# rogeliorjr/DyCON_Paper_Replication

Hardware: AMD Instinct MI355X
Metric: train volumes/sec (96^3 patch) (higher is better)
Workload: dtype bf16

## Files before the change

### dycon_paper_replication_amd/_lib.py

```python
from __future__ import annotations

import ctypes as C
import os

_HERE = os.path.dirname(os.path.abspath(__file__))
LIB_PATH = os.environ.get("DYCON_LIB", os.path.join(_HERE, "libdycon_hip.so"))

F32, BF16 = 0, 1
CONV_1X1, CONV_K3, CONV_K2S2 = 0, 1, 2

P, I, L, F, Z, U64 = C.c_void_p, C.c_int, C.c_longlong, C.c_float, C.c_size_t, C.c_uint64

SIGNATURES = {
    "dycon_version": (I, []),
    "dycon_last_error": (C.c_char_p, []),
    "dycon_bfrag_bytes": (Z, [I, I, I, I]),
    "dycon_pack_bfrag": (I, [P, P, I, I, I, I, I, L, L, L, L, I, P]),
    "dycon_pack_batch": (I, [P, I, I, P]),
    "dycon_pack_tcn": (I, [P, P, I, I, I, I, L, L, L, L, I, P]),
    "dycon_conv_gemm_workspace": (Z, [I, I, I, I, I, I, I, I, I]),
    "dycon_conv_gemm": (I, [P, P, P, P, I, I, I, I, I, I, I, I, I, I, I, P, Z, P]),
    "dycon_conv_gemm_splits": (I, [I, I, I, I, I, I, I, I, I]),
    "dycon_conv_gemm_ex": (I, [P, P, P, P, I, I, I, I, I, I, I, I, I, I, I, P, Z, I, P]),
    "dycon_conv_direct": (I, [P, I, P, P, P, I, I, I, I, I, I, I, I, I, P]),
    "dycon_conv_wgrad_workspace": (Z, [I, I, I, I, I, I, I]),
    "dycon_conv_wgrad": (I, [P, I, P, I, P, P, I, I, I, I, I, I, I, L, L, L, P, Z, P]),
    "dycon_colsum_workspace": (Z, [L, I]),
    "dycon_colsum": (I, [P, I, P, L, I, P, Z, P]),
    "dycon_norm_workspace": (Z, [I, L, I]),
    "dycon_norm_stats": (I, [P, I, I, L, I, I, F, P, P, P, F, P, Z, P]),
    "dycon_norm_fwd": (I, [P, P, I, I, L, I, I, F, P, P, P, I, P, P, P, P, F, P, Z, P]),
    "dycon_norm_fwd_is_fused": (I, [I, L, I, I]),
    "dycon_norm_fwd_slab": (I, [P, I, P, P, P, I, I, L, I, I, F, P, P, P, I, P, P, P]),
    "dycon_norm_apply": (I, [P, P, I, I, L, I, I, P, P, P, I, P, P, P]),
    "dycon_norm_bwd": (I, [P, I, P, P, I, I, L, I, I, P, P, P, I, P, P, P, P, Z, P]),
    "dycon_norm_bwd_ex": (I, [P, I, P, P, I, I, L, I, I, P, P, P, I, P, P, P, I, P, Z, P]),
    "dycon_norm_sum_dparams": (I, [P, I, I, P, P, P]),
    "dycon_norm_head_workspace": (Z, [I, L]),
    "dycon_norm_head_fwd": (I, [P, I, I, L, I, P, P, P, I, P, P, P, P, P]),
    "dycon_norm_head_bwd": (I, [P, P, P, I, I, L, I, P, P, P, I, P, P, P, P, P, Z, P]),
    "dycon_norm_head_dparams": (I, [P, I, L, P, P, P]),
    "dycon_conv_stats_chunks": (I, [I, I, I, I, I, I, I, I]),
    "dycon_conv_gemm_stats": (I, [P, P, P, P, I, I, I, I, I, I, I, P, Z, P]),
    "dycon_norm_fwd_parts": (I, [P, P, I, I, L, I, I, F, P, P, P, I, P, P, P, P, F, P, I, P]),
    "dycon_norm_stats_parts": (I, [I, I, L, I, I, F, P, P, P, F, P, I, P]),
    "dycon_norm_bwd_ab_offset": (Z, [I, L, I]),
    "dycon_norm_bwd_stats": (I, [P, P, I, I, L, I, I, P, P, P, I, P, P, P, P, Z, P]),
    "dycon_first_block_bwd_workspace": (Z, [I, I, I, I]),
    "dycon_first_block_bwd": (I, [P, P, P, I, I, I, I, I, I, P, P, P, I, P, P, P, P, P, L, L, L, P, Z, P]),
    "dycon_conv1_wgrad_normbwd_workspace": (Z, [I, I, I, I]),
    "dycon_conv1_wgrad_normbwd": (I, [P, P, P, I, I, I, I, I, I, P, P, P, I, P, P, P, P, L, L, L, P, Z, P]),
    "dycon_norm_acc_doubles": (Z, [I, L, I]),
    "dycon_norm_fwd_acc": (I, [P, P, I, I, L, I, I, F, P, P, P, I, P, P, P, P, F, P, P]),
    "dycon_norm_bwd_acc": (I, [P, P, P, I, I, L, I, I, P, P, P, I, P, P, P, P, P, Z, P]),
    "dycon_maxpool2_fwd": (I, [P, P, P, I, I, I, I, I, I, P]),
    "dycon_maxpool2_bwd": (I, [P, P, P, I, I, I, I, I, I, P]),
    "dycon_trilinear_fwd": (I, [P, P, I, I, I, I, I, I, I, I, I, I, I, I, P]),
    "dycon_trilinear_bwd": (I, [P, P, I, I, I, I, I, I, I, I, I, I, I, I, P]),
    "dycon_copy_channels": (I, [P, I, I, P, I, I, L, I, I, P]),
    "dycon_relu_fwd": (I, [P, P, P, P, I, I, L, I, P]),
    "dycon_relu_bwd": (I, [P, P, P, P, I, I, L, I, P]),
    "dycon_scale_channels": (I, [P, P, P, I, I, L, I, P]),
    "dycon_mul_mask": (I, [P, P, F, P, I, L, P]),
    "dycon_dropout_philox": (I, [P, P, I, L, F, U64, U64, P]),
    "dycon_channel_mask_philox": (I, [P, L, F, U64, U64, P]),
    "dycon_add_noise": (I, [P, P, P, I, L, F, F, U64, U64, P]),
    "dycon_tanh": (I, [P, I, P, L, P]),
    "dycon_cast": (I, [P, I, P, I, L, P]),
    "dycon_add": (I, [P, P, P, I, L, P]),
    "dycon_seg_losses_fwd": (I, [P, P, P, I, I, I, L, F, P, I, P]),
    "dycon_seg_losses_bwd": (I, [P, P, P, I, I, I, L, F, P, P, I, P, I, P]),
    "dycon_seg_losses_finalize": (I, [P, I, I, L, F, P, P]),
    "dycon_step_loss": (I, [P, P, F, F, F, I, I, P, P, P]),
    "dycon_step_losses": (I, [P, P, I, I, L, F, C.c_double, F, I, F, F, F, I, I, P, P, P]),
    "dycon_softmax_mse_fwd": (I, [P, P, P, L, I, L, I, P]),
    "dycon_softmax_mse_bwd": (I, [P, P, P, P, L, I, L, I, P]),
    "dycon_softmax_kl_fwd": (I, [P, P, L, I, L, I, P, P, P]),
    "dycon_softmax_kl_bwd": (I, [P, P, L, I, L, I, I, P, P, P]),
    "dycon_dice_fwd": (I, [P, P, I, I, L, I, L, I, P, F, P, P, P]),
    "dycon_dice_bwd": (I, [P, P, I, I, L, I, L, I, P, F, P, P, P, P]),
    "dycon_dice1_fwd": (I, [P, P, I, L, I, L, I, P, P, P]),
    "dycon_dice1_bwd": (I, [P, P, I, L, I, L, I, P, P, P, P]),
    "dycon_entropy_fwd": (I, [P, L, I, L, F, P, P, P, P]),
    "dycon_entropy_bwd": (I, [P, L, I, L, F, P, P, P, P]),
    "dycon_sym_mse_fwd": (I, [P, P, L, P, P, P]),
    "dycon_sym_mse_bwd": (I, [P, P, L, P, P, P]),
    "dycon_kl_rows_fwd": (I, [P, L, P, L, L, L, L, I, P, P, P]),
    "dycon_kl_rows_bwd": (I, [P, L, P, L, L, L, L, I, P, P, L, P]),
    "dycon_focal_fwd": (I, [P, P, I, L, I, L, F, P, I, P, P, P]),
    "dycon_focal_bwd": (I, [P, P, I, L, I, L, F, P, I, P, P, P]),
    "dycon_l2norm_fwd": (I, [P, P, P, I, L, I, F, P]),
    "dycon_l2norm_bwd": (I, [P, P, P, P, I, L, I, F, P]),
    "dycon_mask_pool": (I, [P, I, P, I, I, I, I, I, I, I, P]),
    "dycon_fecl_workspace": (Z, [I, I, I]),
    "dycon_fecl_fwd": (I, [P, P, P, P, I, I, I, I, F, F, I, F, F, P, P, P, Z, P]),
    "dycon_fecl_finalize": (I, [P, C.c_double, F, I, P, P]),
    "dycon_set_scalars": (I, [P, I, F, F, F, F, F, F, F, F, P]),
    "dycon_fecl_bwd": (I, [P, P, P, P, I, I, I, I, F, F, I, F, F, P, P, P, P, Z, P]),
    "dycon_fecl_rows_workspace": (Z, [I, I, I]),
    "dycon_fecl_fwd_rows": (I, [P, P, P, P, I, I, I, I, F, F, P, P, Z, Z, P]),
    "dycon_fecl_gambling_finalize": (I, [P, P, I, I, I, I, P, P, P, P, Z, P, Z, P]),
    "dycon_fecl_gambling_grad": (I, [P, P, L, P, P]),
    "dycon_gambling_softmax_fwd": (I, [P, P, L, I, P]),
    "dycon_gambling_softmax_bwd": (I, [P, P, P, L, I, P]),
    "dycon_gambling_uncertainty_fwd": (I, [P, I, I, I, I, I, I, I, P, I, P]),
    "dycon_gambling_uncertainty_bwd": (I, [P, I, I, I, I, I, I, I, P, P, I, P]),
# ... 141 lines not shown
```

### dycon_paper_replication_amd/csrc/conv.hip

```cpp
#include <stdlib.h>

#include "common.h"

typedef float f32x4 __attribute__((ext_vector_type(4)));
typedef __bf16 bf16x8 __attribute__((ext_vector_type(8)));

template <typename T> struct Frag;
template <> struct Frag<float> { static constexpr int G = 4, KC = 16; };
template <> struct Frag<bf16> { static constexpr int G = 8, KC = 32; };

__device__ __forceinline__ void mma(f32x4& acc, const Vec16<float>& a, const Vec16<float>& b) {
    acc = __builtin_amdgcn_mfma_f32_16x16x4f32(a.v.x, b.v.x, acc, 0, 0, 0);
    acc = __builtin_amdgcn_mfma_f32_16x16x4f32(a.v.y, b.v.y, acc, 0, 0, 0);
    acc = __builtin_amdgcn_mfma_f32_16x16x4f32(a.v.z, b.v.z, acc, 0, 0, 0);
    acc = __builtin_amdgcn_mfma_f32_16x16x4f32(a.v.w, b.v.w, acc, 0, 0, 0);
}
__device__ __forceinline__ void mma(f32x4& acc, const Vec16<bf16>& a, const Vec16<bf16>& b) {
    acc = __builtin_amdgcn_mfma_f32_16x16x32_bf16(__builtin_bit_cast(bf16x8, a.v), __builtin_bit_cast(bf16x8, b.v),
                                                  acc, 0, 0, 0);
}

template <int MODE> __device__ __forceinline__ int n_taps() { return MODE == DYCON_CONV_K3 ? 27 : MODE == DYCON_CONV_K2S2 ? 8 : 1; }

template <int MODE>
__device__ __forceinline__ bool src_voxel(int t, int z, int y, int x, int Di, int Hi, int Wi, int& zi, int& yi, int& xi) {
    if (MODE == DYCON_CONV_K3) {
        const int dz = t / 9, dy = (t / 3) % 3, dx = t % 3;
        zi = z + dz - 1; yi = y + dy - 1; xi = x + dx - 1;
        return (unsigned)zi < (unsigned)Di && (unsigned)yi < (unsigned)Hi && (unsigned)xi < (unsigned)Wi;
    } else if (MODE == DYCON_CONV_K2S2) {
        zi = 2 * z + (t >> 2); yi = 2 * y + ((t >> 1) & 1); xi = 2 * x + (t & 1);
        return true;
    } else {
        zi = z; yi = y; xi = x;
        return true;
    }
}

template <typename T>
__global__ void pack_bfrag_kernel(const float* __restrict__ w, T* __restrict__ out, int Tn, int Cin, int N, int N0,
                                  long long s_t, long long s_c, long long s_n1, long long s_n0, int flip, int NT,
                                  long long total) {
    constexpr int G = Frag<T>::G, KC = Frag<T>::KC;
    for (long long i = (long long)blockIdx.x * blockDim.x + threadIdx.x; i < total; i += (long long)gridDim.x * blockDim.x) {
        const int e = (int)(i % G);
        long long q = i / G;
        const int lane = (int)(q % 64);
        q /= 64;
        const int nt = (int)(q % NT);
        const int kc = (int)(q / NT);
        const int k = kc * KC + G * (lane >> 4) + e;
        const int n = nt * 16 + (lane & 15);
        float v = 0.f;
        if (k < Tn * Cin && n < N) {
            int t = k / Cin;
            const int c = k - t * Cin;
            if (flip) t = Tn - 1 - t;
            v = w[t * s_t + c * s_c + (long long)(n / N0) * s_n1 + (long long)(n % N0) * s_n0];
        }
        stf(out + i, v);
    }
}

__global__ void pack_tcn_kernel(const float* __restrict__ w, float* __restrict__ out, int Tn, int Cin, int N, int N0,
                                long long s_t, long long s_c, long long s_n1, long long s_n0, int flip, long long total) {
    for (long long i = (long long)blockIdx.x * blockDim.x + threadIdx.x; i < total; i += (long long)gridDim.x * blockDim.x) {
        const int n = (int)(i % N);
        const long long q = i / N;
        const int c = (int)(q % Cin);
        int t = (int)(q / Cin);
        if (flip) t = Tn - 1 - t;
        out[i] = w[t * s_t + c * s_c + (long long)(n / N0) * s_n1 + (long long)(n % N0) * s_n0];
    }
}

__global__ __launch_bounds__(256) void pack_batch_kernel(const dycon_pack_job_t* __restrict__ jobs) {
    const dycon_pack_job_t jb = jobs[blockIdx.y];
    if (jb.kind == 2) {
        for (long long i = (long long)blockIdx.x * 256 + threadIdx.x; i < jb.total; i += (long long)gridDim.x * 256) {
            const int n = (int)(i % jb.N);
            const long long q = i / jb.N;
            const int c = (int)(q % jb.Cin);
            int t = (int)(q / jb.Cin);
            if (jb.flip) t = jb.T - 1 - t;
            ((float*)jb.out)[i] = jb.w[t * jb.s_t + c * jb.s_c + (long long)(n / jb.N0) * jb.s_n1 + (long long)(n % jb.N0) * jb.s_n0];
// ... 2440 lines not shown
    const ReduceJob j1{bias_part, bias_out, P, bias_part ? Cout : 0, 1, Cout, 0, 0, 1};
    const bool vec = L % 4 == 0 && (!bias_part || Cout % 4 == 0) && ((uintptr_t)part & 15) == 0 && (!bias_part || ((uintptr_t)bias_part & 15) == 0);
    if (vec) {
        const int nb0 = cdiv(L, 128), nb1 = bias_part ? cdiv(Cout, 128) : 0;
        reduce_partials_kernel<4><<<nb0 + nb1, 256, 0, stream>>>(j0, j1, nb0);
    } else {
        const int nb0 = cdiv(L, 32), nb1 = bias_part ? cdiv(Cout, 32) : 0;
        reduce_partials_kernel<1><<<nb0 + nb1, 256, 0, stream>>>(j0, j1, nb0);
    }
}

static void row_grid(int mode, int Di, int Hi, int Wi, int& Do, int& Ho, int& Wo) {
    if (mode == DYCON_CONV_K2S2) { Do = Di / 2; Ho = Hi / 2; Wo = Wi / 2; }
    else { Do = Di; Ho = Hi; Wo = Wi; }
}

extern "C" size_t dycon_bfrag_bytes(int dtype, int T, int Cin, int N) {
    const int KC = dtype == DYCON_BF16 ? 32 : 16, es = dtype == DYCON_BF16 ? 2 : 4;
    const long long nKC = ((long long)T * Cin + KC - 1) / KC, NT = (N + 15) / 16;
    return (size_t)(nKC * NT * 64 * (16 / es) * es);
}

extern "C" int dycon_pack_bfrag(const float* w, void* out, int dtype, int Tn, int Cin, int N, int N0, long long s_t,
                                long long s_c, long long s_n1, long long s_n0, int flip_taps, dycon_stream_t stream) {
    DYCON_REQUIRE(w && out && Tn > 0 && Cin > 0 && N > 0 && N0 > 0, "pack_bfrag: bad arguments");
    DYCON_DISPATCH(dtype, {
        constexpr int G = Frag<T>::G, KC = Frag<T>::KC;
        const int NT = (N + 15) / 16;
        const long long nKC = ((long long)Tn * Cin + KC - 1) / KC;
        const long long total = nKC * NT * 64 * G;
        const int grid = cdiv(total, 256) > 4096 ? 4096 : cdiv(total, 256);
        pack_bfrag_kernel<T><<<grid, 256, 0, stream>>>(w, (T*)out, Tn, Cin, N, N0, s_t, s_c, s_n1, s_n0, flip_taps, NT, total);
    });
    DYCON_LAUNCH_CHECK();
    return DYCON_OK;
}

extern "C" int dycon_pack_tcn(const float* w, float* out, int T, int Cin, int N, int N0, long long s_t, long long s_c,
                              long long s_n1, long long s_n0, int flip_taps, dycon_stream_t stream) {
    DYCON_REQUIRE(w && out && T > 0 && Cin > 0 && N > 0 && N0 > 0, "pack_tcn: bad arguments");
    const long long total = (long long)T * Cin * N;
    pack_tcn_kernel<<<cdiv(total, 256), 256, 0, stream>>>(w, out, T, Cin, N, N0, s_t, s_c, s_n1, s_n0, flip_taps, total);
    DYCON_LAUNCH_CHECK();
    return DYCON_OK;
}

struct SplitK { int splits, kc_per_split; };
static SplitK splitk_plan(int dtype, int mode, int scatter, long long M, int N, int Cin) {
    const int KC = dtype == DYCON_BF16 ? 32 : 16;
    const int Tn = mode == DYCON_CONV_K3 ? 27 : mode == DYCON_CONV_K2S2 ? 8 : 1;
    const int nKC = (Tn * Cin + KC - 1) / KC;
    const long long wgs = ((M + 63) / 64) * (((N + 15) / 16 + NTB - 1) / NTB);
    SplitK p{1, nKC};
    if (scatter || wgs >= 512 || nKC < 16) return p;
    long long s = (1024 + wgs - 1) / wgs;
    if (s > nKC / 6) s = nKC / 6;
    if (s < 2) return p;
    p.kc_per_split = (int)((nKC + s - 1) / s);
    p.splits = (nKC + p.kc_per_split - 1) / p.kc_per_split;
    return p;
}

static bool conv_tile_ok(int dtype, int mode, int scatter, long long DHW, int Cin, int N) {
    return dtype == DYCON_BF16 && mode == DYCON_CONV_K3 && !scatter && Cin % 32 == 0 && N % CT_BN == 0 && Cin >= 64 && DHW < 13824;
}
static SplitK conv_tile_plan(long long M, int N, int Cin) {
    constexpr long long target_wgs = 512;
    const int nKC = 27 * Cin / 32;
    const long long wgs = ((M + CT_BM - 1) / CT_BM) * (N / CT_BN);
    SplitK p{1, nKC};
    if (wgs >= 384) return p;
    long long s = target_wgs / wgs;
    if (s > nKC / 8) s = nKC / 8;
    if (s < 2) return p;
    p.kc_per_split = (int)((nKC + s - 1) / s);
    if (Cin % 64 == 0) p.kc_per_split = (p.kc_per_split + 1) & ~1;
    p.splits = (nKC + p.kc_per_split - 1) / p.kc_per_split;
    return p;
}
static bool conv_halo_ok(int dtype, int mode, int scatter, long long M, long long DHW, int Cin, int N) {
    return conv_tile_ok(dtype, mode, scatter, DHW, Cin, N) && Cin == CH_CIN && conv_tile_plan(M, N, Cin).splits <= CH_MAXS;
}

extern "C" int dycon_pack_batch(const dycon_pack_job_t* jobs_dev, int njobs, int blocks_per_job, dycon_stream_t stream) {
    DYCON_REQUIRE(jobs_dev && njobs > 0 && njobs <= 65535 && blocks_per_job > 0, "pack_batch: bad arguments");
    pack_batch_kernel<<<dim3(blocks_per_job, njobs), 256, 0, stream>>>(jobs_dev);
    DYCON_LAUNCH_CHECK();
    return DYCON_OK;
}

template <typename T, int MODE, bool SC>
static void launch_gemm(const void* x, const void* wf, const float* bias, void* y, int accumulate, int B, int Di, int Hi,
                        int Wi, int Cin, int N, int Cout, float* workspace, int defer_finish, dycon_stream_t stream) {
    int Do, Ho, Wo;
    row_grid(MODE, Di, Hi, Wi, Do, Ho, Wo);
    const long long M = (long long)B * Do * Ho * Wo;
    const int NT = (N + 15) / 16;
    const int Tn = MODE == DYCON_CONV_K3 ? 27 : MODE == DYCON_CONV_K2S2 ? 8 : 1;
    const int nKC = (Tn * Cin + Frag<T>::KC - 1) / Frag<T>::KC;
    const SplitK sk = splitk_plan(sizeof(T) == 2 ? DYCON_BF16 : DYCON_F32, MODE, SC, M, N, Cin);
    const bool split = sk.splits > 1 && workspace != nullptr;
    dim3 grid(cdiv(M, 64), cdiv(NT, NTB), split ? sk.splits : 1);
    conv_gemm_kernel<T, MODE, SC><<<grid, 256, 0, stream>>>((const T*)x, (const T*)wf, bias, (T*)y, B, Di, Hi, Wi, Cin, Do, Ho,
                                                            Wo, N, Cout, NT, nKC, accumulate, split ? workspace : nullptr,
                                                            sk.kc_per_split, split && defer_finish && N % 8 == 0);
    if (split && !defer_finish) {
        long long blocks = (M * N / 4 + 255) / 256;
        if (blocks > 2048) blocks = 2048;
        splitk_finish_kernel<T><<<(int)blocks, 256, 0, stream>>>(workspace, sk.splits, M * N, N, bias, (T*)y, accumulate);
    }
}

extern "C" size_t dycon_conv_gemm_workspace(int dtype, int mode, int scatter, int B, int Di, int Hi, int Wi, int Cin, int N) {
    int Do, Ho, Wo;
    row_grid(mode, Di, Hi, Wi, Do, Ho, Wo);
    const long long M = (long long)B * Do * Ho * Wo;
    if (conv_halo_ok(dtype, mode, scatter, M, (long long)Di * Hi * Wi, Cin, N)) return 0;
    const SplitK sk = conv_tile_ok(dtype, mode, scatter, (long long)Di * Hi * Wi, Cin, N) ? conv_tile_plan(M, N, Cin)
                                                                                       : splitk_plan(dtype, mode, scatter, M, N, Cin);
    return sk.splits > 1 ? (size_t)sk.splits * M * N * sizeof(float) : 0;
}

extern "C" int dycon_conv_gemm_splits(int dtype, int mode, int scatter, int B, int Di, int Hi, int Wi, int Cin, int N) {
    int Do, Ho, Wo;
    row_grid(mode, Di, Hi, Wi, Do, Ho, Wo);
    const long long M = (long long)B * Do * Ho * Wo;
    if (conv_halo_ok(dtype, mode, scatter, M, (long long)Di * Hi * Wi, Cin, N)) return 1;
    const SplitK sk = conv_tile_ok(dtype, mode, scatter, (long long)Di * Hi * Wi, Cin, N) ? conv_tile_plan(M, N, Cin)
                                                                                       : splitk_plan(dtype, mode, scatter, M, N, Cin);
    return sk.splits;
}

extern "C" int dycon_conv_gemm_ex(const void* x, const void* wfrag, const float* bias, void* y, int dtype, int mode,
                                  int scatter, int accumulate, int B, int Di, int Hi, int Wi, int Cin, int N, int Cout,
                                  float* workspace, size_t ws_bytes, int defer_finish, dycon_stream_t stream);

extern "C" int dycon_conv_gemm(const void* x, const void* wfrag, const float* bias, void* y, int dtype, int mode,
                               int scatter, int accumulate, int B, int Di, int Hi, int Wi, int Cin, int N, int Cout,
                               float* workspace, size_t ws_bytes, dycon_stream_t stream) {
    return dycon_conv_gemm_ex(x, wfrag, bias, y, dtype, mode, scatter, accumulate, B, Di, Hi, Wi, Cin, N, Cout, workspace, ws_bytes, 0,
                              stream);
}

static thread_local float* g_stat_part = nullptr;

static bool conv_p32_shape(int dtype, int mode, int scatter, int accumulate, int B, int Di, int Hi, int Wi, int Cin, int Cout) {
    const int nTiles = B * cdiv(Di, CL_TZ) * cdiv(Hi, CL_TY) * cdiv(Wi, CL_TX);
    return dtype == DYCON_BF16 && mode == DYCON_CONV_K3 && !scatter && !accumulate && Cin == 32 && Cout == 32 &&
           (long long)Di * Hi * Wi >= 13824 && nTiles >= 1024;
}
extern "C" int dycon_conv_stats_chunks(int dtype, int mode, int B, int Di, int Hi, int Wi, int Cin, int Cout) {
    const int nTiles = B * cdiv(Di, CL_TZ) * cdiv(Hi, CL_TY) * cdiv(Wi, CL_TX);
    if (dtype == DYCON_BF16 && mode == DYCON_CONV_K3 && Cout == 16 && (Cin == 16 || Cin == 1) && (long long)Di * Hi * Wi >= 13824)
        return 8 * min(cdiv(nTiles, 8), Cin == 16 ? 32 * P16_WGS : 128);
    if (!conv_p32_shape(dtype, mode, 0, 0, B, Di, Hi, Wi, Cin, Cout)) return 0;
    return 8 * min(cdiv(nTiles, 8), 32);
}
extern "C" int dycon_conv_gemm_ex(const void* x, const void* wfrag, const float* bias, void* y, int dtype, int mode,
                                  int scatter, int accumulate, int B, int Di, int Hi, int Wi, int Cin, int N, int Cout,
                                  float* workspace, size_t ws_bytes, int defer_finish, dycon_stream_t stream);
extern "C" int dycon_conv_gemm_stats(const void* x, const void* wfrag, const float* bias, void* y, int dtype, int B, int Di, int Hi,
                                     int Wi, int Cin, int Cout, float* stat_part, size_t stat_bytes, dycon_stream_t stream) {
    const int chunks = dycon_conv_stats_chunks(dtype, DYCON_CONV_K3, B, Di, Hi, Wi, Cin, Cout);
    DYCON_REQUIRE(chunks > 0, "conv_gemm_stats: shape not served (ask dycon_conv_stats_chunks)");
    DYCON_REQUIRE(stat_part && stat_bytes >= (size_t)B * chunks * Cout * 2 * sizeof(float), "conv_gemm_stats: statistics buffer too small");
    g_stat_part = stat_part;
    const int rc = dycon_conv_gemm_ex(x, wfrag, bias, y, dtype, DYCON_CONV_K3, 0, 0, B, Di, Hi, Wi, Cin, Cout, Cout, nullptr, 0, 0, stream);
    g_stat_part = nullptr;
    return rc;
}

extern "C" int dycon_conv_gemm_ex(const void* x, const void* wfrag, const float* bias, void* y, int dtype, int mode,
                                  int scatter, int accumulate, int B, int Di, int Hi, int Wi, int Cin, int N, int Cout,
                                  float* workspace, size_t ws_bytes, int defer_finish, dycon_stream_t stream) {
    DYCON_REQUIRE(x && wfrag && y, "conv_gemm: null pointer");
    DYCON_REQUIRE(!defer_finish || (!accumulate && workspace && dycon_conv_gemm_splits(dtype, mode, scatter, B, Di, Hi, Wi, Cin, N) > 1 &&
                                    ws_bytes >= dycon_conv_gemm_workspace(dtype, mode, scatter, B, Di, Hi, Wi, Cin, N)),
                  "conv_gemm: defer_finish needs a split-K shape, its workspace and no accumulation");
    DYCON_REQUIRE(B > 0 && Di > 0 && Hi > 0 && Wi > 0 && Cin > 0 && N > 0 && Cout > 0, "conv_gemm: bad shape");
    DYCON_REQUIRE(mode >= 0 && mode <= 2, "conv_gemm: bad mode %d", mode);
    const bool first_layer_lds = dtype == DYCON_BF16 && mode == DYCON_CONV_K3 && !scatter && Cin == 1 &&
                                 (Cout == 16 || Cout == 32 || Cout == 64) && (long long)Di * Hi * Wi >= 13824;
    DYCON_REQUIRE(first_layer_lds || Cin % (dtype == DYCON_BF16 ? 8 : 4) == 0, "conv_gemm: Cin=%d not a multiple of the fragment width", Cin);
    DYCON_REQUIRE(N % 16 == 0, "conv_gemm: N=%d not a multiple of 16 (use dycon_conv_direct)", N);
    DYCON_REQUIRE(!scatter || (mode == DYCON_CONV_1X1 && N == 8 * Cout), "conv_gemm: scatter needs mode 1x1 and N == 8*Cout");
    DYCON_REQUIRE(scatter || N == Cout, "conv_gemm: N must equal Cout without scatter");
    DYCON_REQUIRE(mode != DYCON_CONV_K2S2 || (Di % 2 == 0 && Hi % 2 == 0 && Wi % 2 == 0), "conv_gemm: k2s2 needs even dims");
    if (dtype == DYCON_BF16 && mode == DYCON_CONV_K3 && !scatter &&
        ((Cin == 1 && (Cout == 16 || Cout == 32 || Cout == 64)) ||
         ((Cin == 16 || Cin == 48 || Cin % 32 == 0) && (Cout == 16 || Cout == 32 || Cout % 64 == 0 || Cout % 48 == 0))) &&
        (long long)Di * Hi * Wi >= 13824) {
        const int tz = cdiv(Di, CL_TZ), ty = cdiv(Hi, CL_TY), tx = cdiv(Wi, CL_TX);
        const int NT = Cout / 16;
        const int ntb = Cout % 64 == 0 ? CL_NTB64 : (Cout % 48 == 0 ? 3 : NT);
        const int nTiles = B * tz * ty * tx;
        if ((Cin == 16 && Cout == 16) || (Cin == 1 && (Cout == 16 || Cout == 32 || Cout == 64))) {
            const int per_xcd = min(cdiv(nTiles, 8), Cin == 16 ? 32 * P16_WGS : 128);
            const bf16 *xp = (const bf16*)x, *wp = (const bf16*)wfrag;
            bf16* yp = (bf16*)y;
            if (Cin == 16 && accumulate) conv_k3_p16_kernel<P16_DEPTH, true><<<8 * per_xcd, 256, 0, stream>>>(xp, wp, bias, yp, B, Di, Hi, Wi, tz, ty, tx, nTiles);
            else if (Cin == 16 && g_stat_part) conv_k3_p16_kernel<P16_DEPTH, false, true><<<8 * per_xcd, 256, 0, stream>>>(xp, wp, bias, yp, B, Di, Hi, Wi, tz, ty, tx, nTiles, g_stat_part);
            else if (Cin == 16) conv_k3_p16_kernel<P16_DEPTH, false><<<8 * per_xcd, 256, 0, stream>>>(xp, wp, bias, yp, B, Di, Hi, Wi, tz, ty, tx, nTiles);
            else if (Cout == 16 && g_stat_part && !accumulate) conv_k3_c1_kernel<1, true><<<8 * per_xcd, 256, 0, stream>>>(xp, wp, bias, yp, B, Di, Hi, Wi, tz, ty, tx, nTiles, 0, g_stat_part);
            else if (Cout == 16) conv_k3_c1_kernel<1><<<8 * per_xcd, 256, 0, stream>>>(xp, wp, bias, yp, B, Di, Hi, Wi, tz, ty, tx, nTiles, accumulate);
            else if (Cout == 32) conv_k3_c1_kernel<2><<<8 * per_xcd, 256, 0, stream>>>(xp, wp, bias, yp, B, Di, Hi, Wi, tz, ty, tx, nTiles, accumulate);
            else conv_k3_c1_kernel<4><<<8 * per_xcd, 256, 0, stream>>>(xp, wp, bias, yp, B, Di, Hi, Wi, tz, ty, tx, nTiles, accumulate);
            DYCON_LAUNCH_CHECK();
            return DYCON_OK;
        }
        if (Cin == 32 && Cout == 32 && !accumulate && nTiles >= 1024) {
            const int per_xcd = min(cdiv(nTiles, 8), 32);
#define DYCON_P32(STV) conv_k3_p32_kernel<8, STV><<<8 * per_xcd, 64 * 8, 0, stream>>>((const bf16*)x, (const bf16*)wfrag, bias, (bf16*)y, B, Di, Hi, Wi, tz, ty, tx, nTiles, g_stat_part)
            if (g_stat_part) DYCON_P32(true); else DYCON_P32(false);
#undef DYCON_P32
            DYCON_LAUNCH_CHECK();
            return DYCON_OK;
        }
        dim3 grid(nTiles, NT / ntb);
#define DYCON_CL(CKV, NTBV, WMV) \
    conv_k3_lds_kernel<CKV, NTBV, WMV><<<grid, 256, 0, stream>>>((const bf16*)x, (const bf16*)wfrag, bias, (bf16*)y, B, Di, Hi, Wi, Cin, Cout, NT, tz, ty, tx, accumulate)
        if (Cin == 16 || Cin == 48) {
            if (ntb == 1) DYCON_CL(16, 1, 4); else if (ntb == 2) DYCON_CL(16, 2, 4); else if (ntb == 3) DYCON_CL(16, 3, 4); else DYCON_CL(16, 4, 2);
        } else {
            if (ntb == 1) DYCON_CL(32, 1, 4); else if (ntb == 2) DYCON_CL(32, 2, 4); else if (ntb == 3) DYCON_CL(32, 3, 4);
            else if ((long long)nTiles * (NT / ntb) <= 256)
                conv_k3_lds_kernel<32, 4, 4, 8><<<grid, 512, 0, stream>>>((const bf16*)x, (const bf16*)wfrag, bias, (bf16*)y, B, Di, Hi, Wi, Cin, Cout, NT, tz, ty, tx, accumulate);
            else DYCON_CL(32, 4, 2);
        }
#undef DYCON_CL
        DYCON_LAUNCH_CHECK();
        return DYCON_OK;
    }
    if (conv_halo_ok(dtype, mode, scatter, (long long)B * Di * Hi * Wi, (long long)Di * Hi * Wi, Cin, N)) {
        const long long M = (long long)B * Di * Hi * Wi;
        const int tz = cdiv(Di, CH_T), ty = cdiv(Hi, CH_T), tx = cdiv(Wi, CH_T);
        const SplitK sk = conv_tile_plan(M, N, Cin);
        const dim3 grid(B * tz * ty * tx, N / 64);
#define DYCON_CH(NJV) conv_k3_halo_kernel<NJV><<<grid, 64 * CH_NW, 0, stream>>>((const bf16*)x, (const bf16*)wfrag, bias, (bf16*)y, Di, Hi, Wi, N, N / 16, tz, ty, tx, sk.splits, sk.kc_per_split, accumulate)
        if (sk.splits > 2) DYCON_CH(2); else DYCON_CH(1);
#undef DYCON_CH
        DYCON_LAUNCH_CHECK();
        return DYCON_OK;
    }
    if (conv_tile_ok(dtype, mode, scatter, (long long)Di * Hi * Wi, Cin, N)) {
        const long long M = (long long)B * Di * Hi * Wi;
        const int NT = N / 16, nKC = 27 * Cin / 32;
        SplitK sk = conv_tile_plan(M, N, Cin);
        const bool split = sk.splits > 1 && workspace && ws_bytes >= (size_t)sk.splits * M * N * sizeof(float);
        dim3 grid(cdiv(M, CT_BM), N / CT_BN, split ? sk.splits : 1);
        const int layout = split && defer_finish ? 1 : 0;
        if (Cin % 64 == 0 && sk.kc_per_split % 2 == 0)
            conv_k3_tile_kernel<2><<<grid, 256, 0, stream>>>((const bf16*)x, (const bf16*)wfrag, bias, (bf16*)y, split ? workspace : nullptr, B,
                                                             Di, Hi, Wi, Cin, N, NT, nKC, sk.kc_per_split, accumulate, layout);
        else
            conv_k3_tile_kernel<1><<<grid, 256, 0, stream>>>((const bf16*)x, (const bf16*)wfrag, bias, (bf16*)y, split ? workspace : nullptr, B,
                                                             Di, Hi, Wi, Cin, N, NT, nKC, sk.kc_per_split, accumulate, layout);
        DYCON_LAUNCH_CHECK();
        if (split && !defer_finish) {
            long long blocks = (M * N / 4 + 255) / 256;
            if (blocks > 2048) blocks = 2048;
            splitk_finish_kernel<bf16><<<(int)blocks, 256, 0, stream>>>(workspace, sk.splits, M * N, N, bias, (bf16*)y, accumulate);
            DYCON_LAUNCH_CHECK();
        }
        return DYCON_OK;
    }
    float* ws = (workspace && ws_bytes >= dycon_conv_gemm_workspace(dtype, mode, scatter, B, Di, Hi, Wi, Cin, N)) ? workspace : nullptr;
    DYCON_DISPATCH(dtype, {
        if (scatter) launch_gemm<T, DYCON_CONV_1X1, true>(x, wfrag, bias, y, accumulate, B, Di, Hi, Wi, Cin, N, Cout, ws, defer_finish, stream);
        else if (mode == DYCON_CONV_K3) launch_gemm<T, DYCON_CONV_K3, false>(x, wfrag, bias, y, accumulate, B, Di, Hi, Wi, Cin, N, Cout, ws, defer_finish, stream);
        else if (mode == DYCON_CONV_K2S2) launch_gemm<T, DYCON_CONV_K2S2, false>(x, wfrag, bias, y, accumulate, B, Di, Hi, Wi, Cin, N, Cout, ws, defer_finish, stream);
        else launch_gemm<T, DYCON_CONV_1X1, false>(x, wfrag, bias, y, accumulate, B, Di, Hi, Wi, Cin, N, Cout, ws, defer_finish, stream);
    });
    DYCON_LAUNCH_CHECK();
    return DYCON_OK;
}

template <typename TI, typename TO>
static void launch_direct(const void* x, const float* w, const float* bias, void* y, int mode, int accumulate, int B, int Di,
                          int Hi, int Wi, int Cin, int N, dycon_stream_t stream) {
    int Do, Ho, Wo;
    row_grid(mode, Di, Hi, Wi, Do, Ho, Wo);
    const long long M = (long long)B * Do * Ho * Wo;
    const int grid = cdiv(M, 256);
#define DYCON_DIRECT(MODE) \
    conv_direct_kernel<TI, TO, MODE><<<grid, 256, 0, stream>>>((const TI*)x, w, bias, (TO*)y, B, Di, Hi, Wi, Cin, Do, Ho, Wo, N, accumulate)
    if (mode == DYCON_CONV_K3) DYCON_DIRECT(DYCON_CONV_K3);
    else if (mode == DYCON_CONV_K2S2) DYCON_DIRECT(DYCON_CONV_K2S2);
    else DYCON_DIRECT(DYCON_CONV_1X1);
#undef DYCON_DIRECT
}

extern "C" int dycon_conv_direct(const void* x, int x_dtype, const float* w_tcn, const float* bias, void* y, int y_dtype,
                                 int mode, int accumulate, int B, int Di, int Hi, int Wi, int Cin, int N,
                                 dycon_stream_t stream) {
    DYCON_REQUIRE(x && w_tcn && y, "conv_direct: null pointer");
    DYCON_REQUIRE(B > 0 && Di > 0 && Hi > 0 && Wi > 0 && Cin > 0 && N > 0, "conv_direct: bad shape");
    DYCON_REQUIRE(mode >= 0 && mode <= 2, "conv_direct: bad mode %d", mode);
    if (mode == DYCON_CONV_1X1) {
        const long long M = (long long)B * Di * Hi * Wi;
        long long blocks = (M + 255) / 256;
        if (blocks > 4096) blocks = 4096;
        if (Cin == 16 && N == 2 && y_dtype == DYCON_F32 && !accumulate) {
            if (x_dtype == DYCON_F32) head_1x1_fwd_kernel<float, 16, 2><<<(int)blocks, 256, 0, stream>>>((const float*)x, w_tcn, bias, (float*)y, M);
            else head_1x1_fwd_kernel<bf16, 16, 2><<<(int)blocks, 256, 0, stream>>>((const bf16*)x, w_tcn, bias, (float*)y, M);
            DYCON_LAUNCH_CHECK();
            return DYCON_OK;
        }
        if (Cin == 2 && N == 16 && x_dtype == DYCON_F32 && !bias) {
            if (y_dtype == DYCON_F32) head_1x1_bwd_kernel<float, 2, 16><<<(int)blocks, 256, 0, stream>>>((const float*)x, w_tcn, (float*)y, M, accumulate);
            else head_1x1_bwd_kernel<bf16, 2, 16><<<(int)blocks, 256, 0, stream>>>((const float*)x, w_tcn, (bf16*)y, M, accumulate);
            DYCON_LAUNCH_CHECK();
            return DYCON_OK;
        }
    }
    if (x_dtype == DYCON_F32 && y_dtype == DYCON_F32) launch_direct<float, float>(x, w_tcn, bias, y, mode, accumulate, B, Di, Hi, Wi, Cin, N, stream);
    else if (x_dtype == DYCON_BF16 && y_dtype == DYCON_F32) launch_direct<bf16, float>(x, w_tcn, bias, y, mode, accumulate, B, Di, Hi, Wi, Cin, N, stream);
    else if (x_dtype == DYCON_F32 && y_dtype == DYCON_BF16) launch_direct<float, bf16>(x, w_tcn, bias, y, mode, accumulate, B, Di, Hi, Wi, Cin, N, stream);
    else if (x_dtype == DYCON_BF16 && y_dtype == DYCON_BF16) launch_direct<bf16, bf16>(x, w_tcn, bias, y, mode, accumulate, B, Di, Hi, Wi, Cin, N, stream);
    else { dycon_set_error("conv_direct: bad dtypes %d %d", x_dtype, y_dtype); return DYCON_ERR_INVALID; }
    DYCON_LAUNCH_CHECK();
    return DYCON_OK;
}

struct WgradPlan { bool mfma; int splits; long long rows_per_split; int L; };
static WgradPlan wgrad_plan(int mode, int B, int Di, int Hi, int Wi, int Cin, int Cout) {
    int Do, Ho, Wo;
    row_grid(mode, Di, Hi, Wi, Do, Ho, Wo);
    const long long M = (long long)B * Do * Ho * Wo;
    const int Tn = mode == DYCON_CONV_K3 ? 27 : mode == DYCON_CONV_K2S2 ? 8 : 1;
    WgradPlan p;
    p.L = Tn * Cin * Cout;
    p.mfma = (Cin % 16 == 0) && (Cout % 16 == 0);
    if (p.mfma) {
        const long long blocks_xy = (long long)(Cin / 16) * cdiv(Cout, 16 * NTB) * Tn;
        long long want = (2048 + blocks_xy - 1) / blocks_xy;
        long long max_by_rows = (M + 255) / 256;
        long long s = want < 1 ? 1 : want;
        if (s > max_by_rows) s = max_by_rows;
        if (s > 256) s = 256;
        if (s < 1) s = 1;
        long long rps = (M + s - 1) / s;
        rps = (rps + 15) / 16 * 16;
        p.splits = (int)((M + rps - 1) / rps);
        p.rows_per_split = rps;
    } else {
        long long rps = 1024;
        p.splits = (int)((M + rps - 1) / rps);
        p.rows_per_split = rps;
// ... 296 lines not shown
```

### include/dycon_hip.h

```cpp
#ifndef DYCON_HIP_H
#define DYCON_HIP_H

#include <stddef.h>
#include <stdint.h>

#ifdef __cplusplus
extern "C" {
#endif

typedef struct ihipStream_t* dycon_stream_t;

#define DYCON_F32 0
#define DYCON_BF16 1

#define DYCON_OK 0
#define DYCON_ERR_INVALID (-22)
#define DYCON_ERR_LAUNCH (-5)

#define DYCON_CONV_1X1 0
#define DYCON_CONV_K3 1
#define DYCON_CONV_K2S2 2

int dycon_version(void);
const char* dycon_last_error(void);

size_t dycon_bfrag_bytes(int dtype, int T, int Cin, int N);
int dycon_pack_bfrag(const float* w, void* out, int dtype, int T, int Cin, int N, int N0,
                     long long s_t, long long s_c, long long s_n1, long long s_n0, int flip_taps,
                     dycon_stream_t stream);
typedef struct {
    const float* w;
    void* out;
    long long s_t, s_c, s_n1, s_n0, total;
    int kind, T, Cin, N, N0, flip, NT, pad_;
} dycon_pack_job_t;
int dycon_pack_batch(const dycon_pack_job_t* jobs_dev, int njobs, int blocks_per_job, dycon_stream_t stream);
int dycon_pack_tcn(const float* w, float* out, int T, int Cin, int N, int N0, long long s_t,
                   long long s_c, long long s_n1, long long s_n0, int flip_taps, dycon_stream_t stream);

size_t dycon_conv_gemm_workspace(int dtype, int mode, int scatter, int B, int Di, int Hi, int Wi,
                                 int Cin, int N);
int dycon_conv_gemm(const void* x, const void* wfrag, const float* bias, void* y, int dtype,
                    int mode, int scatter, int accumulate, int B, int Di, int Hi, int Wi, int Cin,
                    int N, int Cout, float* workspace, size_t ws_bytes, dycon_stream_t stream);
int dycon_conv_gemm_splits(int dtype, int mode, int scatter, int B, int Di, int Hi, int Wi, int Cin, int N);
int dycon_conv_gemm_ex(const void* x, const void* wfrag, const float* bias, void* y, int dtype,
                       int mode, int scatter, int accumulate, int B, int Di, int Hi, int Wi, int Cin,
                       int N, int Cout, float* workspace, size_t ws_bytes, int defer_finish,
                       dycon_stream_t stream);
int dycon_conv_direct(const void* x, int x_dtype, const float* w_tcn, const float* bias, void* y,
                      int y_dtype, int mode, int accumulate, int B, int Di, int Hi, int Wi, int Cin,
                      int N, dycon_stream_t stream);

size_t dycon_conv_wgrad_workspace(int mode, int B, int Di, int Hi, int Wi, int Cin, int Cout);
int dycon_conv_wgrad(const void* x, int x_dtype, const void* gy, int g_dtype, float* dw, float* dbias,
                     int mode, int B, int Di, int Hi, int Wi, int Cin, int Cout, long long s_t,
                     long long s_c, long long s_n, float* workspace, size_t ws_bytes,
                     dycon_stream_t stream);

size_t dycon_colsum_workspace(long long rows, int C);
int dycon_colsum(const void* x, int dtype, float* out, long long rows, int C, float* workspace,
                 size_t ws_bytes, dycon_stream_t stream);

size_t dycon_norm_workspace(int Nb, long long V, int C);
int dycon_norm_stats(const void* x, int dtype, int Nb, long long V, int C, int G, float eps,
                     float* stats, float* running_mean, float* running_var, float momentum,
                     float* workspace, size_t ws_bytes, dycon_stream_t stream);
int dycon_norm_fwd(const void* x, void* y, int dtype, int Nb, long long V, int C, int G, float eps,
                   float* stats, const float* gamma, const float* beta, int relu, const void* skip,
                   const float* chan_scale, float* running_mean, float* running_var, float momentum,
                   float* workspace, size_t ws_bytes, dycon_stream_t stream);
int dycon_norm_fwd_is_fused(int dtype, long long V, int C, int G);
int dycon_norm_fwd_slab(const float* slab, int splits, const float* conv_bias, void* x_out, void* y,
                        int dtype, int Nb, long long V, int C, int G, float eps, float* stats,
                        const float* gamma, const float* beta, int relu, const void* skip,
                        const float* chan_scale, dycon_stream_t stream);
int dycon_norm_apply(const void* x, void* y, int dtype, int Nb, long long V, int C, int G,
                     const float* stats, const float* gamma, const float* beta, int relu,
                     const void* skip, const float* chan_scale, dycon_stream_t stream);
int dycon_norm_bwd(const void* src, int from_y, const void* gy, void* gx, int dtype, int Nb,
                   long long V, int C, int G, const float* stats, const float* gamma,
                   const float* beta, int relu, const float* chan_scale, float* dgamma, float* dbeta,
                   float* workspace, size_t ws_bytes, dycon_stream_t stream);
int dycon_norm_bwd_ex(const void* src, int from_y, const void* gy, void* gx, int dtype, int Nb,
                      long long V, int C, int G, const float* stats, const float* gamma,
                      const float* beta, int relu, const float* chan_scale, float* dgamma, float* dbeta,
                      int defer_dparams, float* workspace, size_t ws_bytes, dycon_stream_t stream);
int dycon_norm_sum_dparams(const float* workspace, int Nb, int C, float* dgamma, float* dbeta,
                           dycon_stream_t stream);
size_t dycon_norm_head_workspace(int Nb, long long V);
int dycon_norm_head_fwd(const void* x, int dtype, int Nb, long long V, int G, const float* stats, const float* gamma,
                        const float* beta, int relu, const float* chan_scale, const float* head_w, const float* head_b,
                        float* logits, dycon_stream_t stream);
int dycon_norm_head_bwd(const void* x, const float* g_logits, void* gx, int dtype, int Nb, long long V, int G,
                        const float* stats, const float* gamma, const float* beta, int relu, const float* chan_scale,
                        const float* head_w, float* dgamma, float* dbeta, float* workspace, size_t ws_bytes,
                        dycon_stream_t stream);
int dycon_norm_head_dparams(const float* workspace, int Nb, long long V, float* d_head_w, float* d_head_b,
                            dycon_stream_t stream);
int dycon_conv_stats_chunks(int dtype, int mode, int B, int Di, int Hi, int Wi, int Cin, int Cout);
int dycon_norm_stats_parts(int dtype, int Nb, long long V, int C, int G, float eps, float* stats, float* running_mean,
                           float* running_var, float momentum, const float* part, int chunks, dycon_stream_t stream);
int dycon_conv_gemm_stats(const void* x, const void* wfrag, const float* bias, void* y, int dtype, int B, int Di, int Hi,
                          int Wi, int Cin, int Cout, float* stat_part, size_t stat_bytes, dycon_stream_t stream);
int dycon_norm_fwd_parts(const void* x, void* y, int dtype, int Nb, long long V, int C, int G, float eps, float* stats,
                         const float* gamma, const float* beta, int relu, const void* skip, const float* chan_scale,
                         float* running_mean, float* running_var, float momentum, const float* part, int chunks,
                         dycon_stream_t stream);
size_t dycon_norm_bwd_ab_offset(int Nb, long long V, int C);
int dycon_norm_bwd_stats(const void* src, const void* gy, int dtype, int Nb, long long V, int C, int G, const float* stats,
                         const float* gamma, const float* beta, int relu, const float* chan_scale, float* dgamma,
                         float* dbeta, float* workspace, size_t ws_bytes, dycon_stream_t stream);
size_t dycon_first_block_bwd_workspace(int B, int D, int H, int W);
int dycon_first_block_bwd(const void* x, const void* z, const void* gy, int B, int D, int H, int W, int Nb, int G,
                          const float* stats, const float* gamma, const float* beta, int relu, const float* chan_scale,
                          float* dgamma, float* dbeta, float* dw, float* dbias, long long s_t, long long s_c, long long s_n,
                          float* workspace, size_t ws_bytes, dycon_stream_t stream);
size_t dycon_conv1_wgrad_normbwd_workspace(int B, int D, int H, int W);
int dycon_conv1_wgrad_normbwd(const void* x, const void* z, const void* gy, int B, int D, int H, int W, int Nb, int G,
                              const float* stats, const float* gamma, const float* beta, int relu, const float* chan_scale,
                              const float* ab, float* dw, float* dbias, long long s_t, long long s_c, long long s_n,
                              float* workspace, size_t ws_bytes, dycon_stream_t stream);
size_t dycon_norm_acc_doubles(int Nb, long long V, int C);
int dycon_norm_fwd_acc(const void* x, void* y, int dtype, int Nb, long long V, int C, int G, float eps,
                       float* stats, const float* gamma, const float* beta, int relu, const void* skip,
                       const float* chan_scale, float* running_mean, float* running_var, float momentum,
                       double* acc, dycon_stream_t stream);
int dycon_norm_bwd_acc(const void* src, const void* gy, void* gx, int dtype, int Nb, long long V, int C,
                       int G, const float* stats, const float* gamma, const float* beta, int relu,
                       const float* chan_scale, float* dgamma, float* dbeta, double* acc, float* workspace,
                       size_t ws_bytes, dycon_stream_t stream);

// ... 173 lines not shown
```

Before: 905.1.

## Add in-workgroup split-K kernel for bf16 k2s2 strided convolutions

Adds a dedicated kernel for bf16 2x2x2 stride-2 convolutions. The K dimension is split across waves inside a single workgroup and the partial sums are reduced through LDS, which removes the global fp32 split-K workspace and the separate finish kernel. The kernel double-buffers its loads and writes coalesced bf16 output via an LDS transpose. The old split-K path stays reachable through a new explicit entry point, and the in-workgroup path is limited to at most 5 splits and to shapes with enough tiles.

```diff
diff --git a/dycon_paper_replication_amd/_lib.py b/dycon_paper_replication_amd/_lib.py
--- a/dycon_paper_replication_amd/_lib.py
+++ b/dycon_paper_replication_amd/_lib.py
@@ -22,6 +22,8 @@
     "dycon_conv_gemm": (I, [P, P, P, P, I, I, I, I, I, I, I, I, I, I, I, P, Z, P]),
     "dycon_conv_gemm_splits": (I, [I, I, I, I, I, I, I, I, I]),
     "dycon_conv_gemm_ex": (I, [P, P, P, P, I, I, I, I, I, I, I, I, I, I, I, P, Z, I, P]),
+    "dycon_conv_gemm_splitk_workspace": (Z, [I, I, I, I, I, I, I, I]),
+    "dycon_conv_gemm_splitk": (I, [P, P, P, P, I, I, I, I, I, I, I, I, I, P, Z, P]),
     "dycon_conv_direct": (I, [P, I, P, P, P, I, I, I, I, I, I, I, I, I, P]),
     "dycon_conv_wgrad_workspace": (Z, [I, I, I, I, I, I, I]),
     "dycon_conv_wgrad": (I, [P, I, P, I, P, P, I, I, I, I, I, I, I, L, L, L, P, Z, P]),
diff --git a/dycon_paper_replication_amd/csrc/conv.hip b/dycon_paper_replication_amd/csrc/conv.hip
--- a/dycon_paper_replication_amd/csrc/conv.hip
+++ b/dycon_paper_replication_amd/csrc/conv.hip
@@ -1,6 +1,7 @@
 #include <stdlib.h>
 
 #include "common.h"
+#include "conv_k2s2.h"
 
 typedef float f32x4 __attribute__((ext_vector_type(4)));
 typedef __bf16 bf16x8 __attribute__((ext_vector_type(8)));
@@ -2607,6 +2608,12 @@
     return conv_tile_ok(dtype, mode, scatter, DHW, Cin, N) && Cin == CH_CIN && conv_tile_plan(M, N, Cin).splits <= CH_MAXS;
 }
 
+static bool conv_k2s2_inwg_ok(int dtype, int mode, int scatter, long long M, int Cin, int N) {
+    if (dtype != DYCON_BF16 || mode != DYCON_CONV_K2S2 || scatter || Cin % 32 != 0 || N % 64 != 0) return false;
+    const SplitK sk = splitk_plan(dtype, mode, scatter, M, N, Cin);
+    return sk.splits > 1 && sk.splits <= KI_MAXS && ((M + 63) / 64) * (N / 64) >= 32 && M * 8 * Cin < (1LL << 30);
+}
+
 extern "C" int dycon_pack_batch(const dycon_pack_job_t* jobs_dev, int njobs, int blocks_per_job, dycon_stream_t stream) {
     DYCON_REQUIRE(jobs_dev && njobs > 0 && njobs <= 65535 && blocks_per_job > 0, "pack_batch: bad arguments");
     pack_batch_kernel<<<dim3(blocks_per_job, njobs), 256, 0, stream>>>(jobs_dev);
@@ -2640,7 +2647,7 @@
     int Do, Ho, Wo;
     row_grid(mode, Di, Hi, Wi, Do, Ho, Wo);
     const long long M = (long long)B * Do * Ho * Wo;
-    if (conv_halo_ok(dtype, mode, scatter, M, (long long)Di * Hi * Wi, Cin, N)) return 0;
+    if (conv_halo_ok(dtype, mode, scatter, M, (long long)Di * Hi * Wi, Cin, N) || conv_k2s2_inwg_ok(dtype, mode, scatter, M, Cin, N)) return 0;
     const SplitK sk = conv_tile_ok(dtype, mode, scatter, (long long)Di * Hi * Wi, Cin, N) ? conv_tile_plan(M, N, Cin)
                                                                                        : splitk_plan(dtype, mode, scatter, M, N, Cin);
     return sk.splits > 1 ? (size_t)sk.splits * M * N * sizeof(float) : 0;
@@ -2650,10 +2657,35 @@
     int Do, Ho, Wo;
     row_grid(mode, Di, Hi, Wi, Do, Ho, Wo);
     const long long M = (long long)B * Do * Ho * Wo;
-    if (conv_halo_ok(dtype, mode, scatter, M, (long long)Di * Hi * Wi, Cin, N)) return 1;
+    if (conv_halo_ok(dtype, mode, scatter, M, (long long)Di * Hi * Wi, Cin, N) || conv_k2s2_inwg_ok(dtype, mode, scatter, M, Cin, N)) return 1;
     const SplitK sk = conv_tile_ok(dtype, mode, scatter, (long long)Di * Hi * Wi, Cin, N) ? conv_tile_plan(M, N, Cin)
                                                                                        : splitk_plan(dtype, mode, scatter, M, N, Cin);
     return sk.splits;
+}
+
+extern "C" size_t dycon_conv_gemm_splitk_workspace(int dtype, int mode, int B, int Di, int Hi, int Wi, int Cin, int N) {
+    int Do, Ho, Wo;
+    row_grid(mode, Di, Hi, Wi, Do, Ho, Wo);
+    const long long M = (long long)B * Do * Ho * Wo;
+    const SplitK sk = splitk_plan(dtype, mode, 0, M, N, Cin);
+    return sk.splits > 1 ? (size_t)sk.splits * M * N * sizeof(float) : 0;
+}
+extern "C" int dycon_conv_gemm_splitk(const void* x, const void* wfrag, const float* bias, void* y, int dtype, int mode, int accumulate,
+                                      int B, int Di, int Hi, int Wi, int Cin, int N, float* workspace, size_t ws_bytes,
+                                      dycon_stream_t stream) {
+    DYCON_REQUIRE(x && wfrag && y && workspace, "conv_gemm_splitk: null pointer");
+    DYCON_REQUIRE(B > 0 && Di > 0 && Hi > 0 && Wi > 0 && mode >= 0 && mode <= 2, "conv_gemm_splitk: bad shape");
+    DYCON_REQUIRE(Cin % (dtype == DYCON_BF16 ? 8 : 4) == 0 && N % 16 == 0, "conv_gemm_splitk: Cin=%d / N=%d not fragment multiples", Cin, N);
+    DYCON_REQUIRE(mode != DYCON_CONV_K2S2 || (Di % 2 == 0 && Hi % 2 == 0 && Wi % 2 == 0), "conv_gemm_splitk: k2s2 needs even dims");
+    const size_t need = dycon_conv_gemm_splitk_workspace(dtype, mode, B, Di, Hi, Wi, Cin, N);
+    DYCON_REQUIRE(need > 0 && ws_bytes >= need, "conv_gemm_splitk: not a split-K shape, or workspace too small");
+    DYCON_DISPATCH(dtype, {
+        if (mode == DYCON_CONV_K3) launch_gemm<T, DYCON_CONV_K3, false>(x, wfrag, bias, y, accumulate, B, Di, Hi, Wi, Cin, N, N, workspace, 0, stream);
+        else if (mode == DYCON_CONV_K2S2) launch_gemm<T, DYCON_CONV_K2S2, false>(x, wfrag, bias, y, accumulate, B, Di, Hi, Wi, Cin, N, N, workspace, 0, stream);
+        else launch_gemm<T, DYCON_CONV_1X1, false>(x, wfrag, bias, y, accumulate, B, Di, Hi, Wi, Cin, N, N, workspace, 0, stream);
+    });
+    DYCON_LAUNCH_CHECK();
+    return DYCON_OK;
 }
 
 extern "C" int dycon_conv_gemm_ex(const void* x, const void* wfrag, const float* bias, void* y, int dtype, int mode,
@@ -2789,6 +2821,13 @@
         }
         return DYCON_OK;
     }
+    if (mode == DYCON_CONV_K2S2 && conv_k2s2_inwg_ok(dtype, mode, scatter, (long long)B * (Di / 2) * (Hi / 2) * (Wi / 2), Cin, N)) {
+        const long long M = (long long)B * (Di / 2) * (Hi / 2) * (Wi / 2);
+        const SplitK sk = splitk_plan(dtype, mode, scatter, M, N, Cin);
+        conv_k2s2_inwg_launch(x, wfrag, bias, y, M, Di, Hi, Wi, Cin, N, sk.splits, sk.kc_per_split, accumulate, stream);
+        DYCON_LAUNCH_CHECK();
+        return DYCON_OK;
+    }
     float* ws = (workspace && ws_bytes >= dycon_conv_gemm_workspace(dtype, mode, scatter, B, Di, Hi, Wi, Cin, N)) ? workspace : nullptr;
     DYCON_DISPATCH(dtype, {
         if (scatter) launch_gemm<T, DYCON_CONV_1X1, true>(x, wfrag, bias, y, accumulate, B, Di, Hi, Wi, Cin, N, Cout, ws, defer_finish, stream);
diff --git a/dycon_paper_replication_amd/csrc/conv_k2s2.h b/dycon_paper_replication_amd/csrc/conv_k2s2.h
--- /dev/null
+++ b/dycon_paper_replication_amd/csrc/conv_k2s2.h
@@ -0,0 +1,7 @@
+#pragma once
+#include "common.h"
+
+constexpr int KI_MAXS = 5;
+
+void conv_k2s2_inwg_launch(const void* x, const void* wfrag, const float* bias, void* y, long long M, int Di, int Hi, int Wi, int Cin,
+                           int N, int S, int kc_per_split, int accumulate, dycon_stream_t stream);
diff --git a/dycon_paper_replication_amd/csrc/conv_k2s2.hip b/dycon_paper_replication_amd/csrc/conv_k2s2.hip
--- /dev/null
+++ b/dycon_paper_replication_amd/csrc/conv_k2s2.hip
@@ -0,0 +1,115 @@
+#include "conv_k2s2.h"
+
+typedef float f32x4 __attribute__((ext_vector_type(4)));
+typedef __bf16 bf16x8 __attribute__((ext_vector_type(8)));
+
+constexpr int KI_RED_BYTES = KI_MAXS * 8 * 1024;
+constexpr int KI_OP = 64 + 8;
+
+template <int NJ>
+__global__ __launch_bounds__(NJ == 1 ? 512 : 640) __attribute__((amdgpu_waves_per_eu(NJ == 1 ? 5 : 4, NJ == 1 ? 5 : 4)))
+void conv_k2s2_inwg_kernel(const bf16* __restrict__ X, const bf16* __restrict__ Wf, const float* __restrict__ bias, bf16* __restrict__ Y,
+                           long long M, int Di, int Hi, int Wi, int Cin, int N, int NT, int nKC, int S, int kc_per_split, int accumulate) {
+    constexpr int WPS = 4 / NJ;
+    __shared__ __attribute__((aligned(16))) unsigned char lds[KI_RED_BYTES + 64 * KI_OP * 2];
+    unsigned short* ot = reinterpret_cast<unsigned short*>(lds + KI_RED_BYTES);
+    const int tid = threadIdx.x, lane = tid & 63;
+    const int wave = __builtin_amdgcn_readfirstlane(tid >> 6);
+    const int r = lane & 15, kg = lane >> 4;
+    const int nt0 = blockIdx.y * 4;
+    const long long m0 = (long long)blockIdx.x * 64;
+    const int zs = wave / WPS, cg = wave % WPS;
+    const int k0 = zs * kc_per_split, k1 = zs < S ? min(nKC, k0 + kc_per_split) : k0;
+    const int Do = Di >> 1, Ho = Hi >> 1, Wo = Wi >> 1;
+
+    unsigned aoff[4];
+#pragma unroll
+    for (int m = 0; m < 4; ++m) {
+        unsigned q = (unsigned)m0 + m * 16 + r;
+        if (q >= (unsigned)M) q = 0;
+        const unsigned xo = q % Wo; q /= Wo;
+        const unsigned yo = q % Ho; q /= Ho;
+        const unsigned zo = q % Do, bo = q / Do;
+        aoff[m] = ((((bo * Di + 2 * zo) * Hi + 2 * yo) * Wi + 2 * xo) * Cin + 8 * kg) * 2u;
+    }
+    const unsigned boff = lane * 16u;
+    struct Stage { uint4 a[4], b[NJ]; };
+    auto request = [&](int kc, Stage& st) {
+        const int t = (kc * 32) / Cin, c = kc * 32 - t * Cin;
+        const char* xs = reinterpret_cast<const char*>(X) + ((((long long)(t >> 2) * Hi + ((t >> 1) & 1)) * Wi + (t & 1)) * Cin + c) * 2;
+#pragma unroll
+        for (int m = 0; m < 4; ++m) st.a[m] = *reinterpret_cast<const uint4*>(xs + aoff[m]);
+        const char* ws = reinterpret_cast<const char*>(Wf) + ((long long)kc * NT + nt0 + cg * NJ) * 1024;
+#pragma unroll
+        for (int j = 0; j < NJ; ++j) st.b[j] = *reinterpret_cast<const uint4*>(ws + j * 1024 + boff);
+    };
+    f32x4 acc[4][NJ];
+#pragma unroll
+    for (int m = 0; m < 4; ++m)
+#pragma unroll
+        for (int j = 0; j < NJ; ++j) acc[m][j] = f32x4{0.f, 0.f, 0.f, 0.f};
+    auto compute = [&](const Stage& st) {
+#pragma unroll
+        for (int m = 0; m < 4; ++m)
+#pragma unroll
+            for (int j = 0; j < NJ; ++j)
+                acc[m][j] = __builtin_amdgcn_mfma_f32_16x16x32_bf16(__builtin_bit_cast(bf16x8, st.a[m]), __builtin_bit_cast(bf16x8, st.b[j]), acc[m][j], 0, 0, 0);
+    };
+    if (k0 < k1) {
+        Stage s0, s1;
+        int kc = k0;
+        request(kc, s0);
+        if (kc + 1 < k1) request(kc + 1, s1);
+        while (true) {
+            compute(s0);
+            if (kc + 2 < k1) request(kc + 2, s0);
+            if (++kc >= k1) break;
+            compute(s1);
+            if (kc + 2 < k1) request(kc + 2, s1);
+            if (++kc >= k1) break;
+        }
+    }
+
+    float* red = reinterpret_cast<float*>(lds);
+    const int rm = wave >> 1, rj = wave & 1;
+#pragma unroll
+    for (int h = 0; h < 2; ++h) {
+        if (k0 < k1) {
+#pragma unroll
+            for (int j = 0; j < NJ; ++j) {
+                const int jt = cg * NJ + j;
+                if ((jt >> 1) != h) continue;
+#pragma unroll
+                for (int m = 0; m < 4; ++m)
+                    *reinterpret_cast<f32x4*>(red + zs * 2048 + ((m * 2 + (jt & 1)) * 64 + lane) * 4) = acc[m][j];
+            }
+        }
+        __syncthreads();
+        if (wave < 8) {
+            const int col = (2 * h + rj) * 16 + r;
+            const int n = nt0 * 16 + col;
+            const float bv = bias ? bias[n] : 0.f;
+            f32x4 o = f32x4{bv, bv, bv, bv};
+            for (int z = 0; z < S; ++z) o += *reinterpret_cast<const f32x4*>(red + z * 2048 + tid * 4);
+#pragma unroll
+            for (int i = 0; i < 4; ++i) {
+                const int row = rm * 16 + kg * 4 + i;
+                float v = o[i];
+                if (accumulate && m0 + row < M) v += ldf(Y + (m0 + row) * N + n);
+                ot[row * KI_OP + col] = f32_to_bf16_bits(v);
+            }
+        }
+        __syncthreads();
+    }
+    const int row = tid >> 3, pc = tid & 7;
+    if (wave < 8 && m0 + row < M)
+        *reinterpret_cast<uint4*>(Y + (m0 + row) * N + nt0 * 16 + pc * 8) = *reinterpret_cast<const uint4*>(ot + row * KI_OP + pc * 8);
+}
+
+void conv_k2s2_inwg_launch(const void* x, const void* wfrag, const float* bias, void* y, long long M, int Di, int Hi, int Wi, int Cin,
+                           int N, int S, int kc_per_split, int accumulate, dycon_stream_t stream) {
+    const dim3 grid((unsigned)((M + 63) / 64), N / 64);
+#define DYCON_KI(NJV, THREADS) conv_k2s2_inwg_kernel<NJV><<<grid, THREADS, 0, stream>>>((const bf16*)x, (const bf16*)wfrag, bias, (bf16*)y, M, Di, Hi, Wi, Cin, N, N / 16, 8 * Cin / 32, S, kc_per_split, accumulate)
+    if (S <= 2) DYCON_KI(1, 512); else DYCON_KI(2, S == 5 ? 640 : 512);
+#undef DYCON_KI
+}
diff --git a/include/dycon_hip.h b/include/dycon_hip.h
--- a/include/dycon_hip.h
+++ b/include/dycon_hip.h
@@ -48,6 +48,10 @@
                        int mode, int scatter, int accumulate, int B, int Di, int Hi, int Wi, int Cin,
                        int N, int Cout, float* workspace, size_t ws_bytes, int defer_finish,
                        dycon_stream_t stream);
+size_t dycon_conv_gemm_splitk_workspace(int dtype, int mode, int B, int Di, int Hi, int Wi, int Cin, int N);
+int dycon_conv_gemm_splitk(const void* x, const void* wfrag, const float* bias, void* y, int dtype, int mode,
+                           int accumulate, int B, int Di, int Hi, int Wi, int Cin, int N, float* workspace,
+                           size_t ws_bytes, dycon_stream_t stream);
 int dycon_conv_direct(const void* x, int x_dtype, const float* w_tcn, const float* bias, void* y,
                       int y_dtype, int mode, int accumulate, int B, int Di, int Hi, int Wi, int Cin,
                       int N, dycon_stream_t stream);
```

After: 906.7 (median of 3 runs). No clear change (+0.2%).
